# Arthur151/ROMP

Measured on NVIDIA H100. Metric: frames/sec 512x512 ROMP-HRNet32 (whole hot path), higher is better.
Workload: dtype bf16

## Files before the change

### romp_b200/_lib.py

```python
from __future__ import annotations

import ctypes as C
import os
import subprocess
import sys

HERE = os.path.dirname(os.path.abspath(__file__))
ROOT = os.path.dirname(HERE)
LIB_PATH = os.path.join(HERE, "lib", "libb200romp.so")
CSRC = os.path.join(HERE, "csrc")
SOURCES = ["net.cu", "conv_simt.cu", "conv_tc.cu", "conv_block_tc.cu", "conv_bottleneck_tc.cu", "conv_stem_tc.cu", "conv1d_tc.cu", "parse.cu", "smpl.cu", "smpl_blend_tc.cu", "project.cu", "pnp.cu", "bev.cu", "pack.cu", "preproc.cu", "temporal.cu", "track.cu", "romp_track.cu", "resnet_ops.cu"]

F32, BF16, U8 = 0, 1, 2
ENGINE_AUTO, ENGINE_SIMT, ENGINE_WGMMA, ENGINE_TF32 = 0, 1, 2, 3
ENGINE_TCGEN05 = ENGINE_WGMMA


class ConvDesc(C.Structure):
    _fields_ = [(n, C.c_int) for n in (
        "in_", "in_c_off", "out", "out_c_off", "res", "res_c_off", "res_broadcast", "cin", "cout",
        "ksize", "stride", "relu", "upsample", "input_norm", "pow_channel", "engine")]


class SumDesc(C.Structure):
    _fields_ = [("out", C.c_int), ("base", C.c_int), ("n_terms", C.c_int), ("term", C.c_int * 4), ("up", C.c_int * 4),
                ("relu", C.c_int), ("term_c_off", C.c_int * 4)]


class BevWeights(C.Structure):
    _fields_ = [(n, C.POINTER(C.c_float)) for n in (
        "center_ref", "cam_ref", "coordmap", "anchors", "embed", "w0", "b0", "w1", "b1", "w2", "b2")]


NVCC_FLAGS = ["-Xcompiler", "-fPIC", "-std=c++17", "-O3", "-lineinfo", "-gencode", "arch=compute_90a,code=sm_90a"]
OBJ_DIR = os.path.join(HERE, "lib", "obj")


def _nvcc():
    return os.environ.get("NVCC", "/usr/local/cuda/bin/nvcc")


def nvcc_command(out_path=LIB_PATH):
    return [_nvcc(), "-shared"] + NVCC_FLAGS + ["-o", out_path] + [os.path.join(CSRC, s) for s in SOURCES]


def _headers_mtime():
    hs = [os.path.join(CSRC, f) for f in os.listdir(CSRC) if f.endswith((".cuh", ".h"))]
    hs.append(os.path.join(ROOT, "include", "b200romp.h"))
    return max(os.path.getmtime(h) for h in hs)


def needs_build():
    if not os.path.exists(LIB_PATH):
        return True
    t = os.path.getmtime(LIB_PATH)
    deps = [os.path.join(CSRC, f) for f in os.listdir(CSRC)] + [os.path.join(ROOT, "include", "b200romp.h")]
    return any(os.path.getmtime(d) > t for d in deps)


def build(force=False, verbose=True):
    if not force and not needs_build():
        return LIB_PATH
    from concurrent.futures import ThreadPoolExecutor
    os.makedirs(OBJ_DIR, exist_ok=True)
# ... 143 lines not shown
```

### romp_b200/csrc/conv_tc.cuh

```cuda
#pragma once
#include <cuda.h>

#include <string>
#include <vector>

#include "common.cuh"

namespace b200romp {

struct S2Maps {
  CUtensorMap m[4];
};

struct TcConvPlan {
  int kind = 0;
  int cin = 0, cout = 0, nt = 0;
  int eb = 2;
  int grid_x = 0, grid_y = 0, stages = 0;
  int smem_bytes = 0;
  void* d_wpack = nullptr;
  CUtensorMap tmap_in;
  S2Maps tmap_s2;
  unsigned kmask = 0xFFFFFFFFu;
  const void* encoded_in = nullptr;
  int encoded_batch = 0;
  void* d_wpack2 = nullptr;
  void* d_wpack3 = nullptr;
  const float* d_bias1 = nullptr;
  const float* d_bias2 = nullptr;
  int fold = 0;
  std::string describe() const;
};

bool tc_conv_supported(const ConvParams& p, int ksize, int stride);
int tc_conv_prepare(const ConvParams& p, int ksize, int stride, const float* w_oihw, int sm_count, TcConvPlan* plan,
                    std::vector<void*>* allocs);
int tc_conv_launch(const TcConvPlan& plan, const ConvParams& p, cudaStream_t stream);
bool tc_conv1d_supported(const ConvParams& p);
int tc_conv1d_prepare(const ConvParams& p, const float* w_oi3, int sm_count, TcConvPlan* plan, std::vector<void*>* allocs);
int tc_conv1d_launch(TcConvPlan& plan, const ConvParams& p, cudaStream_t stream);
bool tc_stem_supported(const ConvParams& p, int ksize, int stride);
int tc_stem_prepare(const ConvParams& p, const float* w_oihw, int sm_count, TcConvPlan* plan, std::vector<void*>* allocs);
int tc_stem_launch(const TcConvPlan& plan, const ConvParams& p, cudaStream_t stream);
bool tc_block_supported(const ConvParams& p, bool fold);
int tc_block_prepare(const ConvParams& p, const float* w1_oihw, const float* b1, const float* w2_oihw, int sm_count,
                     TcConvPlan* plan, std::vector<void*>* allocs);
int tc_block_launch(const TcConvPlan& plan, const ConvParams& p, cudaStream_t stream);
struct BottleneckMids {
  __nv_bfloat16* t1 = nullptr;
  __nv_bfloat16* t2 = nullptr;
  int t1_C = 0, t2_C = 0;
};
bool tc_bottleneck_supported(const ConvParams& p);
int tc_bottleneck_prepare(const ConvParams& p, const float* w1_oihw, const float* b1, const float* w2_oihw, const float* b2,
                          const float* w3_oihw, int sm_count, TcConvPlan* plan, std::vector<void*>* allocs);
int tc_bottleneck_launch(const TcConvPlan& plan, const ConvParams& p, const BottleneckMids& mids, cudaStream_t stream);

}
```

### romp_b200/csrc/net.cu

```cuda
#include <stdarg.h>
#include <stdlib.h>
#include <string.h>

#include <algorithm>
#include <array>
#include <map>
#include <mutex>
#include <vector>

#include "common.cuh"
#include "conv_tc.cuh"

namespace b200romp {

static thread_local std::string g_last_error;

void set_error(const char* fmt, ...) {
  char buf[1024];
  va_list ap;
  va_start(ap, fmt);
  vsnprintf(buf, sizeof(buf), fmt, ap);
  va_end(ap);
  g_last_error = buf;
}

void* upload(const void* host, size_t bytes, std::vector<void*>* allocs) {
  void* d = nullptr;
  cudaError_t e = cudaMalloc(&d, bytes);
  if (e == cudaSuccess) {
    allocs->push_back(d);
    e = cudaMemcpy(d, host, bytes, cudaMemcpyHostToDevice);
  }
  if (e != cudaSuccess) {
    set_error("upload of %zu bytes failed: %s", bytes, cudaGetErrorString(e));
    return nullptr;
  }
  return d;
}

struct Tensor {
  int H, W, C, dtype, nchw, external;
  void* ptr = nullptr;
  bool constant = false;
  int first_def = -1, last_use = -1;
  size_t frame_bytes() const { return (size_t)H * W * C * dtype_size(dtype); }
};

enum class Kernel { Sum, MaxPool, Simt, Generic7x7, Deconv4x4, Wgmma, WgmmaStem, WgmmaConv1d, WgmmaBlock, WgmmaBottleneck };

struct Conv {
  b200romp_conv_desc d;
  std::vector<float> w, b;
  bool stored = false;
};

struct Op {
  Kernel kernel = Kernel::Simt;
  b200romp_sum_desc sum;
  b200romp_conv_desc d;
  std::vector<Conv> parts;
  float* d_w_simt = nullptr;
  float* d_bias = nullptr;
  int coutPad = 0;
  TcConvPlan tc;
  int lane = 0;
};

static std::vector<int> op_outputs(const Op& op) {
  std::vector<int> o{op.d.out};
  for (size_t k = 0; k + 1 < op.parts.size(); ++k)
    if (op.parts[k].stored) o.push_back(op.parts[k].d.out);
  return o;
}

static bool on_wgmma(Kernel k) {
  return k == Kernel::Wgmma || k == Kernel::WgmmaStem || k == Kernel::WgmmaConv1d || k == Kernel::WgmmaBlock || k == Kernel::WgmmaBottleneck;
}

}

using namespace b200romp;

struct b200romp_net {
  int device = 0;
  int sm_count = 132;
  bool finalized = false;
  int max_batch = 0;
  std::vector<Tensor> tensors;
  std::vector<Op> ops;
  std::vector<void*> device_allocs;
  char* workspace = nullptr;
  size_t workspace_bytes = 0;
  struct GraphKey {
    int batch;
    std::vector<void*> ext;
    bool operator<(const GraphKey& o) const { return batch != o.batch ? batch < o.batch : ext < o.ext; }
  };
  std::map<GraphKey, cudaGraphExec_t> graphs;
  bool use_graph = true;
  static constexpr int kLanes = 4;
  cudaStream_t lane_stream[kLanes] = {nullptr, nullptr, nullptr, nullptr};
  std::vector<cudaEvent_t> op_done;
  cudaEvent_t fork_ev = nullptr;
  bool use_lanes = false;
};

static int fill_params(const b200romp_net* net, const Op& op, int batch, bool allow_unbound, ConvParams* out) {
  const b200romp_conv_desc& d = op.d;
  const Tensor& ti = net->tensors[d.in];
  const Tensor& to = net->tensors[d.out];
  ConvParams p;
  memset(&p, 0, sizeof(p));
  p.in = ti.ptr; p.out = to.ptr;
  p.w = op.d_w_simt; p.bias = op.d_bias;
  p.B = batch;
  p.Hin = ti.H; p.Win = ti.W; p.in_C = ti.C; p.in_c_off = d.in_c_off; p.cin = d.cin;
  conv_out_hw(d.ksize, d.stride, ti.H, ti.W, &p.Hout, &p.Wout);
  p.out_C = to.C; p.out_c_off = d.out_c_off; p.cout = d.cout; p.coutPad = op.coutPad;
  p.up = d.upsample;
  if (d.res >= 0) {
    const Tensor& tr = net->tensors[d.res];
    p.res = tr.ptr; p.res_C = tr.C; p.res_c_off = op.d.res_c_off; p.res_broadcast = d.res_broadcast;
    p.res_dtype = tr.dtype;
  }
  p.relu = d.relu; p.pow_channel = d.pow_channel; p.out_nchw = to.nchw;
  p.in_dtype = ti.dtype; p.out_dtype = to.dtype; p.input_norm = d.input_norm;
  if (op.tc.fold) {
    p.Win /= 2; p.Wout /= 2;
    p.in_C *= 2; p.cin *= 2; p.out_C *= 2; p.cout *= 2; p.res_C *= 2;
  }
  if (!allow_unbound && (!p.in || !p.out)) {
    set_error("op uses an unbound tensor (in=%d out=%d)", d.in, d.out);
    return B200ROMP_ESTATE;
  }
  *out = p;
  return B200ROMP_OK;
}

static int validate_desc(const std::vector<Tensor>& T, const b200romp_conv_desc& d) {
  const int res_c_off = d.res_c_off;
  auto ok_id = [&](int id) { return id >= 0 && id < (int)T.size(); };
  B2R_REQUIRE(ok_id(d.in) && ok_id(d.out) && (d.res == -1 || ok_id(d.res)), "conv: bad tensor id");
  B2R_REQUIRE((d.ksize == 1 || d.ksize == 3 || d.ksize == 7 || (d.ksize == 13 && d.stride == 1 && d.upsample == 1) ||
               (d.ksize == 42 && d.stride == 2 && d.upsample == 1)) && (d.stride == 1 || d.stride == 2),
              "conv: ksize/stride unsupported");
  B2R_REQUIRE(d.upsample == 1 || d.upsample == 2 || d.upsample == 4 || d.upsample == 8, "conv: upsample must be 1,2,4,8");
  const Tensor& ti = T[d.in];
  const Tensor& to = T[d.out];
  B2R_REQUIRE(!ti.nchw, "conv: NCHW inputs unsupported");
  B2R_REQUIRE(d.cin > 0 && d.in_c_off >= 0 && d.in_c_off + d.cin <= ti.C, "conv: input channel slice out of range");
  B2R_REQUIRE(d.cout > 0 && d.out_c_off >= 0 && d.out_c_off + d.cout <= to.C, "conv: output channel slice out of range");
  int Ho, Wo;
  conv_out_hw(d.ksize, d.stride, ti.H, ti.W, &Ho, &Wo);
  B2R_REQUIRE(Ho * d.upsample == to.H && Wo * d.upsample == to.W, "conv: output tensor is %dx%d, op produces %dx%d",
              to.H, to.W, Ho * d.upsample, Wo * d.upsample);
  B2R_REQUIRE(ti.dtype != B200ROMP_U8 || d.input_norm || d.ksize == 7, "conv: u8 input requires input_norm (or the 7x7 stem)");
  B2R_REQUIRE(to.dtype != B200ROMP_U8, "conv: u8 output unsupported");
  B2R_REQUIRE(!to.nchw || to.dtype == B200ROMP_F32, "conv: NCHW output must be fp32");
  if (d.res >= 0) {
    const Tensor& tr = T[d.res];
    B2R_REQUIRE(tr.H == to.H && tr.W == to.W && !tr.nchw && tr.dtype != B200ROMP_U8, "conv: residual shape/dtype mismatch");
    B2R_REQUIRE(res_c_off >= 0 && res_c_off + d.cout <= tr.C, "conv: residual channel slice out of range");
  }
  return B200ROMP_OK;
}

extern "C" {

int b200romp_version(void) { return B200ROMP_VERSION; }
const char* b200romp_last_error(void) { return g_last_error.c_str(); }
// ... 112 lines not shown
  B2R_REQUIRE(to.H == (ti.H + 2 - 3) / 2 + 1 && to.W == (ti.W + 2 - 3) / 2 + 1, "add_maxpool: output must be %dx%d", (ti.H - 1) / 2 + 1, (ti.W - 1) / 2 + 1);
  Op op;
  op.kernel = Kernel::MaxPool;
  memset(&op.d, 0, sizeof(op.d));
  memset(&op.sum, 0, sizeof(op.sum));
  op.d.in = in; op.d.out = out; op.d.res = -1;
  net->ops.push_back(std::move(op));
  return (int)net->ops.size() - 1;
}

static int fill_sum_params(b200romp_net* net, const Op& op, int batch, SumParams* out) {
  SumParams p;
  memset(&p, 0, sizeof(p));
  const Tensor& to = net->tensors[op.sum.out];
  const Tensor& tb = net->tensors[op.sum.base];
  B2R_REQUIRE(to.ptr && tb.ptr, "sum op: unbound tensor");
  p.base = tb.ptr; p.base_dt = tb.dtype; p.out = to.ptr; p.out_dt = to.dtype;
  p.n_terms = op.sum.n_terms;
  for (int k = 0; k < p.n_terms; ++k) {
    const Tensor& tt = net->tensors[op.sum.term[k]];
    B2R_REQUIRE(tt.ptr, "sum op: unbound term tensor");
    p.term[k] = tt.ptr; p.term_dt[k] = tt.dtype; p.up[k] = op.sum.up[k];
    p.term_C[k] = tt.C; p.term_c_off[k] = op.sum.term_c_off[k];
  }
  p.B = batch; p.H = to.H; p.W = to.W; p.C = to.C; p.relu = op.sum.relu;
  *out = p;
  return B200ROMP_OK;
}

static int enqueue_op(b200romp_net* net, Op& op, int batch, cudaStream_t stream) {
  ConvParams p;
  if (op.kernel != Kernel::Sum && op.kernel != Kernel::MaxPool) {
    int rc = fill_params(net, op, batch, false, &p);
    if (rc) return rc;
  }
  switch (op.kernel) {
    case Kernel::Sum: {
      SumParams sp;
      int rc = fill_sum_params(net, op, batch, &sp);
      return rc ? rc : launch_fuse_sum(sp, stream);
    }
    case Kernel::MaxPool: {
      const Tensor& ti = net->tensors[op.d.in];
      const Tensor& to = net->tensors[op.d.out];
      B2R_REQUIRE(ti.ptr && to.ptr, "maxpool op: unbound tensor");
      return launch_maxpool3x3s2(ti.ptr, to.ptr, ti.dtype, batch, ti.H, ti.W, ti.C, stream);
    }
    case Kernel::Simt: return launch_conv_simt(p, op.d.ksize, op.d.stride, stream);
    case Kernel::Generic7x7: return launch_conv_generic(p, 7, op.d.stride, stream);
    case Kernel::Deconv4x4: return launch_deconv4x4s2(p, stream);
    case Kernel::Wgmma: return tc_conv_launch(op.tc, p, stream);
    case Kernel::WgmmaStem: return tc_stem_launch(op.tc, p, stream);
    case Kernel::WgmmaConv1d: return tc_conv1d_launch(op.tc, p, stream);
    case Kernel::WgmmaBlock: return tc_block_launch(op.tc, p, stream);
    case Kernel::WgmmaBottleneck: {
      BottleneckMids mids;
      auto mid = [&](int k, int* C) -> __nv_bfloat16* {
        if (!op.parts[k].stored) return nullptr;
        const Tensor& t = net->tensors[op.parts[k].d.out];
        *C = t.C;
        return static_cast<__nv_bfloat16*>(t.ptr);
      };
      mids.t1 = mid(0, &mids.t1_C);
      mids.t2 = mid(1, &mids.t2_C);
      return tc_bottleneck_launch(op.tc, p, mids, stream);
    }
  }
  return B200ROMP_EINVAL;
}

static bool fold_eligible(const b200romp_net* net, const Op& op) {
  static const bool off = [] { const char* e = getenv("B200ROMP_TC_NO_FOLD"); return e && e[0] == '1'; }();
  const b200romp_conv_desc& d = op.d;
  const Tensor& ti = net->tensors[d.in];
  const Tensor& to = net->tensors[d.out];
  if (off || d.ksize != 3 || d.stride != 1 || d.upsample != 1 || d.cin != 32 || d.cout != 32) return false;
  if (ti.C != 32 || to.C != 32 || d.in_c_off || d.out_c_off || ti.external || to.external) return false;
  if (ti.dtype != B200ROMP_BF16 || to.dtype != B200ROMP_BF16 || to.nchw || d.pow_channel >= 0 || d.input_norm) return false;
  if (ti.W % 16 != 0 || ti.H % 16 != 0) return false;
  if (d.res >= 0) {
    const Tensor& tr = net->tensors[d.res];
    if (tr.C != 32 || d.res_c_off || d.res_broadcast || tr.dtype != B200ROMP_BF16 || tr.external) return false;
  }
  return true;
}

static void fold_pixel_pairs(std::vector<float>* w, std::vector<float>* b) {
  std::vector<float> w2((size_t)64 * 64 * 9, 0.f), b2(64);
  for (int dx = 0; dx < 2; ++dx)
    for (int co = 0; co < 32; ++co)
      for (int h = 0; h < 2; ++h)
        for (int ci = 0; ci < 32; ++ci)
          for (int ky = 0; ky < 3; ++ky)
            for (int s = -1; s <= 1; ++s) {
              const int kx = 2 * s + h - dx + 1;
              if (kx < 0 || kx > 2) continue;
              w2[(((size_t)(dx * 32 + co) * 64 + h * 32 + ci) * 3 + ky) * 3 + (s + 1)] = (*w)[(((size_t)co * 32 + ci) * 3 + ky) * 3 + kx];
            }
  for (int i = 0; i < 64; ++i) b2[i] = (*b)[i % 32];
  *w = std::move(w2);
  *b = std::move(b2);
}

static unsigned fold_kmask() {
  unsigned m = 0;
  for (int t = 0; t < 9; ++t) {
    const int s = t % 3 - 1;
    if (s != -1) m |= 1u << (t * 2 + 0);
    if (s != +1) m |= 1u << (t * 2 + 1);
  }
  return m;
}

static bool is_bf16_relu_conv(const b200romp_net* net, const Op& op, int ksize, int cin, int cout) {
  const b200romp_conv_desc& d = op.d;
  const Tensor& ti = net->tensors[d.in];
  const Tensor& to = net->tensors[d.out];
  return d.ksize == ksize && d.stride == 1 && d.upsample == 1 && d.relu && !d.input_norm && d.pow_channel < 0 &&
         (d.engine == B200ROMP_ENGINE_AUTO || d.engine == B200ROMP_ENGINE_WGMMA) && ti.dtype == B200ROMP_BF16 &&
         to.dtype == B200ROMP_BF16 && !to.nchw && d.cin == cin && d.cout == cout;
}

static void count_accesses(const b200romp_net* net, std::vector<int>* reads, std::vector<int>* writes) {
  reads->assign(net->tensors.size(), 0);
  writes->assign(net->tensors.size(), 0);
  for (const Op& op : net->ops) {
    ++(*reads)[op.d.in];
    ++(*writes)[op.d.out];
    if (op.kernel == Kernel::Sum)
      for (int k = 0; k < op.sum.n_terms; ++k) ++(*reads)[op.sum.term[k]];
    else if (op.d.res >= 0) ++(*reads)[op.d.res];
  }
}

static bool fusable_intermediate(const b200romp_net* net, const Op& a, const Op& b, const std::vector<int>& writes) {
  const int t = a.d.out;
  const Tensor& tt = net->tensors[t];
  return b.d.in == t && b.d.in_c_off == 0 && a.d.out_c_off == 0 && tt.C == a.d.cout && !tt.external && !tt.constant &&
         writes[t] == 1 && b.d.res != t;
}

struct ChainPattern {
  Kernel kernel;
  std::vector<std::array<int, 3>> convs;
  bool fold;
  bool shared_mids;
  bool (*supported)(const ConvParams& p, bool fold);
};

static void fuse_chains(b200romp_net* net, const ChainPattern& pat) {
  std::vector<int> reads, writes;
  count_accesses(net, &reads, &writes);
  const size_t n = pat.convs.size();
  std::vector<Op> fused;
  fused.reserve(net->ops.size());
  for (size_t i = 0; i < net->ops.size(); ++i) {
    Op* c = &net->ops[i];
    bool ok = i + n <= net->ops.size();
    for (size_t k = 0; ok && k < n; ++k) {
      const std::array<int, 3>& s = pat.convs[k];
      ok = c[k].kernel == Kernel::Simt && is_bf16_relu_conv(net, c[k], s[0], s[1], s[2]) && c[k].lane == c[0].lane &&
           (!pat.fold || fold_eligible(net, c[k]));
      if (ok && k + 1 < n)
        ok = c[k].d.res < 0 && fusable_intermediate(net, c[k], c[k + 1], writes) && (pat.shared_mids || reads[c[k].d.out] == 1);
    }
    if (ok) {
      const b200romp_conv_desc& first = c[0].d;
      const b200romp_conv_desc& last = c[n - 1].d;
      ok = last.res == first.in && last.res_c_off == first.in_c_off && !last.res_broadcast &&
           !net->tensors[first.in].external && !net->tensors[last.out].external;
    }
    if (ok) {
      Op f;
      f.kernel = pat.kernel;
      f.d = c[0].d;
      f.d.cout = c[n - 1].d.cout;
      f.d.out = c[n - 1].d.out;
      f.d.out_c_off = c[n - 1].d.out_c_off;
      f.d.res = c[0].d.in;
      f.d.res_c_off = c[n - 1].d.res_c_off;
      f.tc.fold = pat.fold;
      f.lane = c[0].lane;
      ConvParams p;
      fill_params(net, f, 1, true, &p);
      if (pat.supported(p, pat.fold)) {
        for (size_t k = 0; k < n; ++k) {
          f.parts.push_back(std::move(c[k].parts[0]));
          f.parts.back().stored = k + 1 < n && reads[c[k].d.out] > 1;
        }
        fused.push_back(std::move(f));
        i += n - 1;
        continue;
      }
    }
    fused.push_back(std::move(net->ops[i]));
  }
  net->ops = std::move(fused);
}

static int choose_kernel(const b200romp_net* net, int i, Op& op) {
  const b200romp_conv_desc& d = op.d;
  const Tensor& ti = net->tensors[d.in];
  const Tensor& to = net->tensors[d.out];
  if (d.ksize == 7 || d.ksize == 42) {
    op.kernel = d.ksize == 7 ? Kernel::Generic7x7 : Kernel::Deconv4x4;
    return B200ROMP_OK;
  }
  op.kernel = Kernel::Simt;
  const bool forced = d.engine == B200ROMP_ENGINE_WGMMA;
  const bool stem = ti.dtype == B200ROMP_U8 && d.cin == 3 && d.ksize == 3 && d.stride == 2;
  if (!forced && !(d.engine == B200ROMP_ENGINE_TF32 && ti.dtype == B200ROMP_F32) &&
      !(d.engine == B200ROMP_ENGINE_AUTO && (ti.dtype == B200ROMP_BF16 || stem)))
    return B200ROMP_OK;
  ConvParams p;
  fill_params(net, op, net->max_batch, true, &p);
  if (stem) {
    if (!to.external && d.res < 0 && tc_stem_supported(p, d.ksize, d.stride)) op.kernel = Kernel::WgmmaStem;
  } else if (d.ksize == 13) {
    if (tc_conv1d_supported(p)) op.kernel = Kernel::WgmmaConv1d;
  } else if (!ti.external && tc_conv_supported(p, d.ksize, d.stride)) {
    op.kernel = Kernel::Wgmma;
    op.tc.fold = fold_eligible(net, op);
  }
  if (forced && op.kernel == Kernel::Simt) {
    set_error("op %d: tensor-core engine forced but shape unsupported", i);
    return B200ROMP_EINVAL;
  }
  return B200ROMP_OK;
}

static int prepare_op(b200romp_net* net, Op& op) {
  if (op.parts.empty()) return B200ROMP_OK;
  const b200romp_conv_desc& d = op.d;
  std::vector<std::vector<float>> w, b;
  for (Conv& c : op.parts) {
    w.push_back(std::move(c.w));
    b.push_back(std::move(c.b));
    if (op.tc.fold) fold_pixel_pairs(&w.back(), &b.back());
  }
  std::vector<float> bias = b.back();
  op.coutPad = ((int)bias.size() + 63) / 64 * 64;
  bias.resize(op.coutPad, 0.f);
  op.d_bias = static_cast<float*>(upload(bias.data(), bias.size() * sizeof(float), &net->device_allocs));
  if (!op.d_bias) return B200ROMP_ECUDA;
  ConvParams p;
  fill_params(net, op, net->max_batch, true, &p);
  switch (op.kernel) {
    case Kernel::Simt:
    case Kernel::Generic7x7:
    case Kernel::Deconv4x4: {
      const int taps = conv_taps(d.ksize);
      std::vector<float> packed((size_t)taps * d.cin * op.coutPad, 0.f);
      for (int co = 0; co < d.cout; ++co)
        for (int ci = 0; ci < d.cin; ++ci)
          for (int t = 0; t < taps; ++t)
            packed[((size_t)t * d.cin + ci) * op.coutPad + co] =
                d.ksize == 42 ? w[0][((size_t)ci * d.cout + co) * taps + t] : w[0][((size_t)co * d.cin + ci) * taps + t];
      op.d_w_simt = static_cast<float*>(upload(packed.data(), packed.size() * sizeof(float), &net->device_allocs));
      return op.d_w_simt ? B200ROMP_OK : B200ROMP_ECUDA;
    }
    case Kernel::Wgmma:
      if (op.tc.fold) op.tc.kmask = fold_kmask();
      return tc_conv_prepare(p, d.ksize, d.stride, w[0].data(), net->sm_count, &op.tc, &net->device_allocs);
    case Kernel::WgmmaStem: return tc_stem_prepare(p, w[0].data(), net->sm_count, &op.tc, &net->device_allocs);
    case Kernel::WgmmaConv1d: return tc_conv1d_prepare(p, w[0].data(), net->sm_count, &op.tc, &net->device_allocs);
    case Kernel::WgmmaBlock:
      return tc_block_prepare(p, w[0].data(), b[0].data(), w[1].data(), net->sm_count, &op.tc, &net->device_allocs);
    case Kernel::WgmmaBottleneck:
      return tc_bottleneck_prepare(p, w[0].data(), b[0].data(), w[1].data(), b[1].data(), w[2].data(), net->sm_count, &op.tc,
                                   &net->device_allocs);
    default: return B200ROMP_OK;
  }
}

int b200romp_net_finalize(b200romp_net* net, int max_batch) {
  B2R_REQUIRE(net && !net->finalized && max_batch > 0, "finalize: bad arguments");
  B2R_CUDA_OK(cudaSetDevice(net->device));
  fuse_chains(net, {Kernel::WgmmaBlock, {{3, 64, 64}, {3, 64, 64}}, false, false, tc_block_supported});
  fuse_chains(net, {Kernel::WgmmaBlock, {{3, 32, 32}, {3, 32, 32}}, true, false, tc_block_supported});
  fuse_chains(net, {Kernel::WgmmaBottleneck, {{1, 256, 64}, {3, 64, 64}, {1, 64, 256}}, false, true,
                    [](const ConvParams& p, bool) { return tc_bottleneck_supported(p); }});
  const int nT = (int)net->tensors.size(), nO = (int)net->ops.size();
  for (int i = 0; i < nO; ++i) {
    const b200romp_conv_desc& d = net->ops[i].d;
    for (int t : op_outputs(net->ops[i])) {
      Tensor& to = net->tensors[t];
      if (to.first_def < 0) to.first_def = i;
      to.last_use = std::max(to.last_use, i);
    }
    net->tensors[d.in].last_use = std::max(net->tensors[d.in].last_use, i);
    if (d.res >= 0) net->tensors[d.res].last_use = std::max(net->tensors[d.res].last_use, i);
    if (net->ops[i].kernel == Kernel::Sum)
      for (int k = 0; k < net->ops[i].sum.n_terms; ++k) {
        Tensor& tt = net->tensors[net->ops[i].sum.term[k]];
        B2R_REQUIRE(tt.external || tt.constant || (tt.first_def >= 0 && tt.first_def < i), "op %d sums tensor %d before it is written", i, net->ops[i].sum.term[k]);
        tt.last_use = std::max(tt.last_use, i);
      }
  }
  for (int i = 0; i < nO; ++i) {
    const b200romp_conv_desc& d = net->ops[i].d;
    const Tensor& ti = net->tensors[d.in];
    B2R_REQUIRE(ti.external || ti.constant || (ti.first_def >= 0 && ti.first_def < i), "op %d reads tensor %d before it is written", i, d.in);
    if (d.res >= 0) {
      const Tensor& tr = net->tensors[d.res];
      B2R_REQUIRE(tr.external || tr.constant || (tr.first_def >= 0 && tr.first_def < i), "op %d adds tensor %d before it is written", i, d.res);
    }
  }
  struct Buf { size_t bytes; size_t offset; };
  std::vector<Buf> bufs;
  std::multimap<size_t, int> free_bufs;
  std::vector<int> tensor_buf(nT, -1);
  std::vector<std::vector<int>> dies_at(nO);
  for (int t = 0; t < nT; ++t) {
    const Tensor& tt = net->tensors[t];
    if (!tt.external && !tt.constant && tt.first_def >= 0) dies_at[tt.last_use].push_back(t);
  }
  size_t total = 0;
  for (int i = 0; i < nO; ++i) {
    for (int t : op_outputs(net->ops[i])) {
      const Tensor& tt = net->tensors[t];
      if (tt.external || tt.constant || tt.first_def != i) continue;
      const size_t bytes = (tt.frame_bytes() * max_batch + 1023) / 1024 * 1024;
      auto it = free_bufs.find(bytes);
      if (it != free_bufs.end()) {
        tensor_buf[t] = it->second;
        free_bufs.erase(it);
      } else {
        bufs.push_back({bytes, total});
        total += bytes;
        tensor_buf[t] = (int)bufs.size() - 1;
      }
    }
    for (int dead : dies_at[i]) free_bufs.insert({bufs[tensor_buf[dead]].bytes, tensor_buf[dead]});
// ... 171 lines not shown
  const Tensor& t = net->tensors[tensor];
  B2R_REQUIRE(t.ptr != nullptr, "read_tensor: tensor %d has no storage", tensor);
  const size_t bytes = t.frame_bytes() * (t.constant ? 1 : batch);
  B2R_CUDA_OK(cudaMemcpyAsync(dst, t.ptr, bytes, cudaMemcpyDeviceToDevice, (cudaStream_t)stream));
  return B200ROMP_OK;
}

int b200romp_net_describe(b200romp_net* net, char* buf, int len) {
  if (!net || !buf || len <= 0) return B200ROMP_EINVAL;
  std::string s;
  char line[384];
  auto conv_line = [&](size_t i, const b200romp_conv_desc& d, Kernel kernel, const char* bracket) {
    const Tensor& ti = net->tensors[d.in];
    const Tensor& to = net->tensors[d.out];
    snprintf(line, sizeof(line), "op%03zu %s k%d s%d %4d->%-4d in t%d[%dx%dx%d]+%d out t%d[%dx%dx%d]+%d res t%d up%d relu%d%s\n", i,
             on_wgmma(kernel) ? "wgmma  " : "simt   ", d.ksize, d.stride, d.cin, d.cout, d.in, ti.H, ti.W, ti.C, d.in_c_off, d.out,
             to.H, to.W, to.C, d.out_c_off, d.res, d.upsample, d.relu, bracket);
    s += line;
  };
  for (size_t i = 0; i < net->ops.size(); ++i) {
    const Op& op = net->ops[i];
    const b200romp_conv_desc& d = op.d;
    const Tensor& ti = net->tensors[d.in];
    const Tensor& to = net->tensors[d.out];
    switch (op.kernel) {
      case Kernel::MaxPool:
        snprintf(line, sizeof(line), "op%03zu maxpool 3x3 s2 in t%d[%dx%dx%d] out t%d[%dx%dx%d]\n", i, d.in, ti.H, ti.W, ti.C, d.out, to.H, to.W, to.C);
        s += line;
        break;
      case Kernel::Sum: {
        int n = snprintf(line, sizeof(line), "op%03zu sum     out t%d[%dx%dx%d] = relu%d( t%d", i, op.sum.out, to.H, to.W, to.C, op.sum.relu, op.sum.base);
        for (int k = 0; k < op.sum.n_terms; ++k) n += snprintf(line + n, sizeof(line) - n, " + up%d(t%d)", op.sum.up[k], op.sum.term[k]);
        n += snprintf(line + n, sizeof(line) - n, " )");
        bool bound = net->finalized && to.ptr && ti.ptr;
        for (int k = 0; k < op.sum.n_terms; ++k) bound = bound && net->tensors[op.sum.term[k]].ptr;
        SumParams sp;
        if (bound && fill_sum_params(net, op, net->max_batch, &sp) == B200ROMP_OK)
          n += snprintf(line + n, sizeof(line) - n, " [fuse-sum %s]", fuse_sum_kernel_name(sp));
        snprintf(line + n, sizeof(line) - n, "\n");
        s += line;
        break;
      }
      case Kernel::WgmmaBlock: {
        const int mid = op.parts[0].d.out;
        const Tensor& tm = net->tensors[mid];
        snprintf(line, sizeof(line),
                 "op%03zu wgmma   block k3 s1 %d->%d->%d in t%d[%dx%dx%d]+%d mid t%d[%dx%dx%d] out t%d[%dx%dx%d]+%d res t%d+%d up1 relu1 "
                 "bias1 bias2 [tc-block grid %d smem %d%s]\n",
                 i, d.cin, d.cin, d.cout, d.in, ti.H, ti.W, ti.C, d.in_c_off, mid, tm.H, tm.W, tm.C, d.out, to.H, to.W, to.C,
                 d.out_c_off, d.res, d.res_c_off, op.tc.grid_x, op.tc.smem_bytes, op.tc.fold ? " conv1 pixel-pairs conv2 pixel-pairs" : "");
        s += line;
        break;
      }
      case Kernel::WgmmaBottleneck:
        for (size_t k = 0; k < op.parts.size(); ++k) {
          char bracket[96];
          snprintf(bracket, sizeof(bracket), " [tc-bottleneck conv%zu of k1-k3-k1 grid %d smem %d]", k + 1, op.tc.grid_x, op.tc.smem_bytes);
          conv_line(i, op.parts[k].d, op.kernel, bracket);
        }
        break;
      default:
        conv_line(i, d, op.kernel, on_wgmma(op.kernel) ? op.tc.describe().c_str() : "");
    }
  }
  snprintf(line, sizeof(line), "workspace %.1f MiB for max_batch %d\n", net->workspace_bytes / 1048576.0, net->max_batch);
  s += line;
  const int n = (int)std::min<size_t>(s.size(), (size_t)len - 1);
  memcpy(buf, s.data(), n);
  buf[n] = 0;
  return n;
}

int b200romp_net_set_lane(b200romp_net* net, int op, int lane) {
  B2R_REQUIRE(net && !net->finalized && op >= 0 && op < (int)net->ops.size(), "set_lane: bad op id or net already finalized");
  B2R_REQUIRE(lane >= 0 && lane < b200romp_net::kLanes, "set_lane: lane must be 0..%d", b200romp_net::kLanes - 1);
  net->ops[op].lane = lane;
  return B200ROMP_OK;
}

int b200romp_net_num_launches(b200romp_net* net) { return net ? (int)net->ops.size() : 0; }
long long b200romp_net_workspace_bytes(b200romp_net* net) { return net ? (long long)net->workspace_bytes : 0; }

int b200romp_conv2d(const b200romp_conv_desc* d, const float* weight_host, const float* bias_host, const void* in,
                    int in_dtype, int in_H, int in_W, int in_C, void* out, int out_dtype, int out_C, int out_nchw,
                    const void* res, int res_dtype, int batch, b200romp_stream stream) {
  B2R_REQUIRE(d && weight_host && in && out && batch > 0, "conv2d: bad arguments");
  int dev = 0;
  B2R_CUDA_OK(cudaGetDevice(&dev));
  b200romp_net* net = b200romp_net_create(dev);
  if (!net) return B200ROMP_ECUDA;
  int Ho, Wo;
  conv_out_hw(d->ksize, d->stride, in_H, in_W, &Ho, &Wo);
  Ho *= d->upsample; Wo *= d->upsample;
  b200romp_conv_desc dd = *d;
  dd.in = b200romp_net_add_tensor(net, in_H, in_W, in_C, in_dtype, 0, 1);
  dd.out = b200romp_net_add_tensor(net, Ho, Wo, out_C, out_dtype, out_nchw, 1);
  dd.res = -1;
  if (res) dd.res = b200romp_net_add_tensor(net, Ho, Wo, out_C, res_dtype, 0, 1);
  int rc = (dd.in < 0 || dd.out < 0) ? B200ROMP_EINVAL : B200ROMP_OK;
  if (!rc) {
    net->tensors[dd.in].ptr = const_cast<void*>(in);
    net->tensors[dd.out].ptr = out;
    if (res) net->tensors[dd.res].ptr = const_cast<void*>(res);
    net->tensors[dd.in].external = net->tensors[dd.out].external = 0;
    if (res) net->tensors[dd.res].external = 0;
    net->tensors[dd.in].constant = true;
// ... 24 lines not shown
```

Before: 3614.

## Fuse HRNet stem's two stride-2 3x3 convs into one warp-specialized WGMMA kernel

Adds a persistent kernel that loads raw u8 frames via TMA, normalizes and im2cols them in producer warps, runs conv1 (3->64, s2) with WGMMA into a parity-split shared-memory tile, then runs conv2 (64->64, s2) directly from shared memory. The aim is to avoid writing and re-reading the full-resolution 64-channel intermediate in global memory and to save a launch. The chain fuser is generalized to match stride, u8 input and non-residual patterns. The intermediate is still written out when another op reads it. This adds halo recomputation and a large shared-memory footprint that limits the kernel to one block per SM.

```diff
diff --git a/romp_b200/_lib.py b/romp_b200/_lib.py
--- a/romp_b200/_lib.py
+++ b/romp_b200/_lib.py
@@ -9,7 +9,7 @@
 ROOT = os.path.dirname(HERE)
 LIB_PATH = os.path.join(HERE, "lib", "libb200romp.so")
 CSRC = os.path.join(HERE, "csrc")
-SOURCES = ["net.cu", "conv_simt.cu", "conv_tc.cu", "conv_block_tc.cu", "conv_bottleneck_tc.cu", "conv_stem_tc.cu", "conv1d_tc.cu", "parse.cu", "smpl.cu", "smpl_blend_tc.cu", "project.cu", "pnp.cu", "bev.cu", "pack.cu", "preproc.cu", "temporal.cu", "track.cu", "romp_track.cu", "resnet_ops.cu"]
+SOURCES = ["net.cu", "conv_simt.cu", "conv_tc.cu", "conv_block_tc.cu", "conv_bottleneck_tc.cu", "conv_stem_tc.cu", "conv_stem_fused_tc.cu", "conv1d_tc.cu", "parse.cu", "smpl.cu", "smpl_blend_tc.cu", "project.cu", "pnp.cu", "bev.cu", "pack.cu", "preproc.cu", "temporal.cu", "track.cu", "romp_track.cu", "resnet_ops.cu"]
 
 F32, BF16, U8 = 0, 1, 2
 ENGINE_AUTO, ENGINE_SIMT, ENGINE_WGMMA, ENGINE_TF32 = 0, 1, 2, 3
diff --git a/romp_b200/csrc/conv_stem_fused_tc.cu b/romp_b200/csrc/conv_stem_fused_tc.cu
--- /dev/null
+++ b/romp_b200/csrc/conv_stem_fused_tc.cu
@@ -0,0 +1,337 @@
+#include "conv_tc.cuh"
+#include "tc_device.cuh"
+
+namespace b200romp {
+
+namespace {
+
+constexpr int kFsThreads = 384;
+constexpr int kFsRowB = 128;
+constexpr int kFsK1RowB = 64;
+constexpr int kFsMidRows = 576;
+constexpr int kFsW2Bytes = 9 * 64 * kFsRowB;
+constexpr int kFsMidBytes = kFsMidRows * kFsRowB;
+constexpr int kFsA1Bytes = kFsMidRows * kFsK1RowB;
+constexpr int kFsW1Bytes = 64 * kFsK1RowB;
+constexpr int kFsRawRowB = 112;
+constexpr int kFsRawRows = 67;
+constexpr int kFsRawBytes = kFsRawRowB * kFsRawRows;
+constexpr int kFsRawStage = (kFsRawBytes + 127) / 128 * 128;
+constexpr int kFsRing = 2;
+constexpr int kFsSmemBytes = kFsW2Bytes + kFsMidBytes + kFsA1Bytes + kFsW1Bytes + kFsRing * kFsRawStage + 1024  +
+                             1024 ;
+static_assert(kFsSmemBytes <= 227 * 1024, "fused stem does not fit shared memory");
+
+__host__ __device__ constexpr int fs_bh(int i) { return i < 2 ? 17 : 16; }
+__host__ __device__ constexpr int fs_bw(int i) { return (i & 1) ? 8 : 9; }
+__host__ __device__ constexpr int fs_sub_row(int i) { return i == 0 ? 0 : fs_sub_row(i - 1) + (fs_bh(i - 1) * fs_bw(i - 1) + 7) / 8 * 8; }
+static_assert(fs_sub_row(4) == 568, "parity layout rows");
+
+__device__ __forceinline__ bool fs_row(int m, int* yl, int* xl) {
+  const int i = m < fs_sub_row(1) ? 0 : m < fs_sub_row(2) ? 1 : m < fs_sub_row(3) ? 2 : 3;
+  const int r = m - (i == 0 ? fs_sub_row(0) : i == 1 ? fs_sub_row(1) : i == 2 ? fs_sub_row(2) : fs_sub_row(3));
+  const int bw = fs_bw(i), a = r / bw, b = r % bw;
+  const bool ok = m < fs_sub_row(4) && a < fs_bh(i);
+  *yl = ok ? 2 * a + (i < 2 ? 0 : 1) : 0;
+  *xl = ok ? 2 * b + ((i & 1) ? 1 : 0) : 0;
+  return ok;
+}
+
+__device__ __forceinline__ void consumers_bar_sync() { asm volatile("bar.sync 1, 256;" ::: "memory"); }
+
+template <typename T>
+__device__ __forceinline__ T opaque(T v) {
+  uint64_t u = (uint64_t)v;
+  asm volatile("mov.b64 %0, %0;" : "+l"(u));
+  return (T)u;
+}
+__device__ __forceinline__ void stmatrix_x4(uint32_t addr, uint32_t r0, uint32_t r1, uint32_t r2, uint32_t r3) {
+  asm volatile("stmatrix.sync.aligned.m8n8.x4.shared.b16 [%0], {%1, %2, %3, %4};" ::"r"(addr), "r"(r0), "r"(r1), "r"(r2), "r"(r3)
+               : "memory");
+}
+__device__ __forceinline__ uint32_t pack_bf16x2(float a, float b) {
+  const __nv_bfloat162 v = __floats2bfloat162_rn(a, b);
+  return *reinterpret_cast<const uint32_t*>(&v);
+}
+
+}
+
+template <bool STORE_MID>
+__global__ void __launch_bounds__(kFsThreads, 1)
+conv_stem_fused_tc_kernel(const __grid_constant__ CUtensorMap raw_map, const ConvParams p, const uint8_t* __restrict__ w1pack,
+                          const uint8_t* __restrict__ w2pack, const float* __restrict__ bias1, __nv_bfloat16* __restrict__ mid,
+                          int tiles_x, int tiles_y, int num_tiles) {
+  extern __shared__ uint8_t smem_raw[];
+  uint8_t* smem = reinterpret_cast<uint8_t*>((reinterpret_cast<uintptr_t>(smem_raw) + 1023) & ~(uintptr_t)1023);
+  uint8_t* sW2 = smem;
+  uint8_t* sMid = sW2 + kFsW2Bytes;
+  uint8_t* sA1 = sMid + kFsMidBytes;
+  uint8_t* sW1 = sA1 + kFsA1Bytes;
+  uint8_t* sRaw = sW1 + kFsW1Bytes;
+  uint64_t* raw_full = reinterpret_cast<uint64_t*>(sRaw + kFsRing * kFsRawStage);
+  uint64_t* raw_empty = raw_full + kFsRing;
+  uint64_t* w_full = raw_empty + kFsRing;
+  uint64_t* a1_full = w_full + 1;
+  uint64_t* a1_empty = a1_full + 1;
+
+  const int warp = threadIdx.x >> 5, l = threadIdx.x & 31;
+  if (threadIdx.x == 0) {
+    for (int i = 0; i < kFsRing; ++i) {
+      mbar_init(&raw_full[i], 1);
+      mbar_init(&raw_empty[i], 3);
+    }
+    mbar_init(w_full, 1);
+    mbar_init(a1_full, 3);
+    mbar_init(a1_empty, 8);
+    fence_barrier_init();
+  }
+  __syncthreads();
+  pdl_trigger();
+  const int per_frame = tiles_x * tiles_y;
+
+  if (warp == 0) {
+    if (elect_one()) {
+      mbar_arrive_expect_tx(w_full, kFsW1Bytes + kFsW2Bytes);
+      bulk_copy_g2s(sW1, w1pack, kFsW1Bytes, w_full);
+      for (int t = 0; t < 9; ++t) bulk_copy_g2s(sW2 + t * 64 * kFsRowB, w2pack + (size_t)t * 64 * kFsRowB, 64 * kFsRowB, w_full);
+      pdl_wait();
+      const uint64_t pol = l2_policy_stream();
+      int slot = 0;
+      uint32_t phase = 0;
+      for (int tile = blockIdx.x; tile < num_tiles; tile += gridDim.x) {
+        const int n = tile / per_frame, rem = tile % per_frame;
+        const int y0 = (rem / tiles_x) * 16, x0 = (rem % tiles_x) * 8;
+        mbar_wait(&raw_empty[slot], phase ^ 1);
+        mbar_arrive_expect_tx(&raw_full[slot], kFsRawBytes);
+        tma_load_3d(sRaw + slot * kFsRawStage, &raw_map, &raw_full[slot], 12 * x0 - 16, 4 * y0 - 3, n, pol);
+        if (++slot == kFsRing) { slot = 0; phase ^= 1; }
+      }
+    }
+  } else if (warp < 4) {
+    const int pt = threadIdx.x - 32;
+    int slot = 0;
+    uint32_t phase = 0, it = 0;
+    for (int tile = blockIdx.x; tile < num_tiles; tile += gridDim.x, ++it) {
+      const int rem = tile % per_frame;
+      const int y0 = (rem / tiles_x) * 16, x0 = (rem % tiles_x) * 8;
+      mbar_wait(&raw_full[slot], phase);
+      mbar_wait(a1_empty, (it & 1) ^ 1);
+      const uint8_t* raw = sRaw + slot * kFsRawStage;
+#pragma unroll 1
+      for (int m = pt; m < kFsMidRows; m += 96) {
+        int yl, xl;
+        const bool row_valid = fs_row(m, &yl, &xl);
+        const int off = 2 * yl * kFsRawRowB + 7 + 6 * xl;
+        const uint32_t* src = reinterpret_cast<const uint32_t*>(raw + (off & ~3));
+        const int sh = 8 * (off & 3);
+        float v[32];
+#pragma unroll
+        for (int r = 0; r < 3; ++r) {
+          const int iy = 4 * y0 - 3 + 2 * yl + r;
+          const bool row_ok = row_valid && iy >= 0 && iy < p.Hin;
+          const uint32_t* q = src + r * (kFsRawRowB / 4);
+          const uint32_t a0 = q[0], a1 = q[1], a2 = q[2];
+          const uint32_t b[3] = {__funnelshift_r(a0, a1, sh), __funnelshift_r(a1, a2, sh), a2 >> sh};
+#pragma unroll
+          for (int s = 0; s < 3; ++s) {
+            const int ix = 4 * x0 - 3 + 2 * xl + s;
+            const bool ok = row_ok && ix >= 0 && ix < p.Win;
+#pragma unroll
+            for (int c = 0; c < 3; ++c) {
+              const int k = s * 3 + c;
+              const float x = __uint_as_float(__byte_perm(b[k >> 2], 0x4B000000u, 0x7540u | (k & 3)));
+              v[r * 9 + k] = ok ? (x - 8388608.f) - 127.5f : 0.f;
+            }
+          }
+        }
+#pragma unroll
+        for (int k = 27; k < 32; ++k) v[k] = 0.f;
+        uint32_t pk[16];
+#pragma unroll
+        for (int k = 0; k < 16; ++k) pk[k] = pack_bf16x2(v[2 * k], v[2 * k + 1]);
+        uint8_t* a = sA1 + m * kFsK1RowB;
+#pragma unroll
+        for (int q4 = 0; q4 < 4; ++q4)
+          *reinterpret_cast<uint4*>(a + ((q4 ^ ((m >> 1) & 3)) * 16)) = make_uint4(pk[4 * q4], pk[4 * q4 + 1], pk[4 * q4 + 2], pk[4 * q4 + 3]);
+      }
+      fence_proxy_async();
+      __syncwarp();
+      if (l == 0) {
+        mbar_arrive(a1_full);
+        mbar_arrive(&raw_empty[slot]);
+      }
+      if (++slot == kFsRing) { slot = 0; phase ^= 1; }
+    }
+  } else {
+    const int g = (warp >> 2) - 1, w = warp & 3;
+    pdl_wait();
+    mbar_wait(w_full, 0);
+    const int cl = 2 * (l & 3);
+    const int Hmid = 2 * p.Hout, Wmid = 2 * p.Wout;
+    uint32_t it = 0;
+    for (int tile = blockIdx.x; tile < num_tiles; tile += gridDim.x, ++it) {
+      const uint32_t w1_base = opaque(smem_u32(sW1)), w2_base = opaque(smem_u32(sW2)), a1_base = opaque(smem_u32(sA1)),
+                     mid_base = opaque(smem_u32(sMid));
+      const float* b1p = opaque(bias1);
+      const float* b2p = opaque(p.bias);
+      const int n = tile / per_frame, rem = tile % per_frame;
+      const int y0 = (rem / tiles_x) * 16, x0 = (rem % tiles_x) * 8;
+
+      auto issue64 = [&](float (&acc)[32], int blk) {
+        wgmma_fence();
+#pragma unroll
+        for (int k = 0; k < 2; ++k)
+          wgmma_n64(acc, make_smem_desc(a1_base + blk * 64 * kFsK1RowB + k * 32, 8 * kFsK1RowB, kSw64),
+                    make_smem_desc(w1_base + k * 32, 8 * kFsK1RowB, kSw64), k, false);
+        wgmma_commit();
+      };
+      float b1v[16], b1h[8];
+#pragma unroll
+      for (int j = 0; j < 8; ++j) { b1v[2 * j] = __ldg(b1p + 8 * j + cl); b1v[2 * j + 1] = __ldg(b1p + 8 * j + cl + 1); }
+#pragma unroll
+      for (int j = 0; j < 4; ++j) { b1h[2 * j] = __ldg(b1p + 32 * g + 8 * j + cl); b1h[2 * j + 1] = __ldg(b1p + 32 * g + 8 * j + cl + 1); }
+      auto epi = [&](const auto& acc, const auto& bias, int blk, int j0) {
+        constexpr int NJ = sizeof(acc) / (4 * sizeof(float));
+        bool zero[2];
+        size_t gpix[2];
+        bool store[2];
+#pragma unroll
+        for (int e = 0; e < 2; ++e) {
+          int yl, xl;
+          const bool row_valid = fs_row(blk * 64 + 16 * w + (l >> 2) + 8 * e, &yl, &xl);
+          const int my = 2 * y0 - 1 + yl, mx = 2 * x0 - 1 + xl;
+          zero[e] = !row_valid || (unsigned)my >= (unsigned)Hmid || (unsigned)mx >= (unsigned)Wmid;
+          store[e] = row_valid && yl >= 1 && xl >= 1;
+          gpix[e] = ((size_t)n * Hmid + my) * Wmid + mx;
+        }
+        const int q = l >> 3, rr = l & 7;
+        const uint32_t row_addr = mid_base + (uint32_t)((blk * 64 + 16 * w + rr + 8 * (q & 1)) * kFsRowB);
+#pragma unroll
+        for (int j = 0; j < NJ; j += 2) {
+          uint32_t r[4];
+#pragma unroll
+          for (int qq = 0; qq < 4; ++qq) {
+            const int e = qq & 1, jl = j + (qq >> 1), jg = j0 + jl;
+            const float a = fmaxf(acc[4 * jl + 2 * e] + bias[2 * jl], 0.f), b = fmaxf(acc[4 * jl + 2 * e + 1] + bias[2 * jl + 1], 0.f);
+            r[qq] = zero[e] ? 0u : pack_bf16x2(a, b);
+            if constexpr (STORE_MID) {
+              if (store[e]) *reinterpret_cast<uint32_t*>(mid + gpix[e] * 64 + 8 * jg + cl) = r[qq];
+            }
+          }
+          stmatrix_x4(row_addr + (((j0 + j + (q >> 1)) ^ rr) << 4), r[0], r[1], r[2], r[3]);
+        }
+      };
+      float acc0[32], acc1[32], acc_b[16];
+      mbar_wait(a1_full, it & 1);
+      issue64(acc0, 4 * g);
+      issue64(acc1, 4 * g + 1);
+      wgmma_wait<1>();
+      consumers_bar_sync();
+      epi(acc0, b1v, 4 * g, 0);
+      issue64(acc0, 4 * g + 2);
+      wgmma_wait<1>();
+      epi(acc1, b1v, 4 * g + 1, 0);
+      issue64(acc1, 4 * g + 3);
+      wgmma_wait<1>();
+      epi(acc0, b1v, 4 * g + 2, 0);
+      wgmma_fence();
+#pragma unroll
+      for (int k = 0; k < 2; ++k)
+        wgmma_n32(acc_b, make_smem_desc(a1_base + 8 * 64 * kFsK1RowB + k * 32, 8 * kFsK1RowB, kSw64),
+                  make_smem_desc(w1_base + 32 * g * kFsK1RowB + k * 32, 8 * kFsK1RowB, kSw64), k, false);
+      wgmma_commit();
+      wgmma_wait<1>();
+      epi(acc1, b1v, 4 * g + 3, 0);
+      wgmma_wait<0>();
+      if (l == 0) mbar_arrive(a1_empty);
+      epi(acc_b, b1h, 8, 4 * g);
+      fence_proxy_async();
+      consumers_bar_sync();
+
+      float acc2[32];
+#pragma unroll
+      for (int j = 0; j < 32; ++j) acc2[j] = 0.f;
+      wgmma_fence();
+#pragma unroll
+      for (int tap = 0; tap < 9; ++tap) {
+        const int r = tap / 3, s = tap % 3;
+        const int sub = (r != 1 ? 0 : 2) + (s != 1 ? 0 : 1);
+        const int bw = fs_bw(sub);
+        const uint32_t a_tap = mid_base + (uint32_t)((fs_sub_row(sub) + (r == 2 ? bw : 0) + (s == 2 ? 1 : 0) + 8 * g * bw) * kFsRowB);
+        const uint32_t b_tap = w2_base + (uint32_t)(tap * 64 * kFsRowB);
+#pragma unroll
+        for (int k = 0; k < 4; ++k)
+          wgmma_n64(acc2, make_smem_desc(a_tap + k * 32, bw * kFsRowB, kSw128), make_smem_desc(b_tap + k * 32, 8 * kFsRowB, kSw128),
+                    (tap | k) != 0, false);
+      }
+      wgmma_commit();
+      wgmma_wait<0>();
+
+      __nv_bfloat16* out = reinterpret_cast<__nv_bfloat16*>(p.out);
+#pragma unroll
+      for (int e = 0; e < 2; ++e) {
+        const size_t pix = ((size_t)n * p.Hout + y0 + 8 * g + 2 * w + e) * p.Wout + x0 + (l >> 2);
+        __nv_bfloat162* o = reinterpret_cast<__nv_bfloat162*>(out + pix * p.out_C + p.out_c_off + cl);
+#pragma unroll
+        for (int j = 0; j < 8; ++j) {
+          const int c = 8 * j + cl;
+          o[4 * j] = __floats2bfloat162_rn(fmaxf(acc2[4 * j + 2 * e] + __ldg(b2p + c), 0.f),
+                                           fmaxf(acc2[4 * j + 2 * e + 1] + __ldg(b2p + c + 1), 0.f));
+        }
+      }
+    }
+  }
+}
+
+bool tc_stem_fused_supported(const ConvParams& p) {
+  return p.cin == 3 && p.in_C == 3 && p.in_c_off == 0 && p.cout == 64 && p.in_dtype == B200ROMP_U8 && p.input_norm &&
+         p.out_dtype == B200ROMP_BF16 && !p.out_nchw && p.up == 1 && p.res == nullptr && p.relu && p.pow_channel < 0 &&
+         p.out_C % 8 == 0 && p.out_c_off % 8 == 0 && p.Hout % 16 == 0 && p.Wout % 8 == 0 && p.Hout * 4 == p.Hin &&
+         p.Wout * 4 == p.Win && (p.Win * 3) % 16 == 0;
+}
+
+int tc_stem_fused_prepare(const ConvParams& p, const float* w1_oihw, const float* b1, const float* w2_oihw, int sm_count,
+                          TcConvPlan* plan, std::vector<void*>* allocs) {
+  plan->kind = 34;
+  plan->eb = 2;
+  plan->cin = 3;
+  plan->cout = plan->nt = 64;
+  plan->grid_x = sm_count;
+  plan->grid_y = 1;
+  plan->stages = kFsRing;
+  plan->smem_bytes = kFsSmemBytes;
+  std::vector<float> wk((size_t)64 * 32, 0.f);
+  for (int co = 0; co < 64; ++co)
+    for (int c = 0; c < 3; ++c)
+      for (int r = 0; r < 3; ++r)
+        for (int s = 0; s < 3; ++s)
+          wk[(size_t)co * 32 + r * 9 + s * 3 + c] = w1_oihw[(((size_t)co * 3 + c) * 3 + r) * 3 + s] * (2.0f / 255.0f);
+  int rc = tc_pack_weights(wk.data(), 32, 64, 1, 64, &plan->d_wpack, allocs, kFsK1RowB, 2);
+  if (!rc) rc = tc_pack_weights(w2_oihw, 64, 64, 9, 64, &plan->d_wpack2, allocs, kFsRowB, 2);
+  if (rc) return rc;
+  plan->d_bias1 = static_cast<const float*>(upload(b1, 64 * sizeof(float), allocs));
+  if (!plan->d_bias1) return B200ROMP_ECUDA;
+  B2R_CUDA_OK(cudaFuncSetAttribute(conv_stem_fused_tc_kernel<false>, cudaFuncAttributeMaxDynamicSharedMemorySize, kFsSmemBytes));
+  B2R_CUDA_OK(cudaFuncSetAttribute(conv_stem_fused_tc_kernel<true>, cudaFuncAttributeMaxDynamicSharedMemorySize, kFsSmemBytes));
+  return B200ROMP_OK;
+}
+
+int tc_stem_fused_launch(const TcConvPlan& plan, const ConvParams& p, __nv_bfloat16* mid, cudaStream_t stream) {
+  B2R_REQUIRE((reinterpret_cast<uintptr_t>(p.in) & 15) == 0 && (p.Win * 3) % 16 == 0,
+              "conv_stem_fused_tc: frames must be 16 B aligned with a row pitch that is a multiple of 16 B");
+  CUtensorMap raw;
+  const cuuint64_t gdim[3] = {(cuuint64_t)p.Win * 3, (cuuint64_t)p.Hin, (cuuint64_t)p.B};
+  const cuuint64_t gstr[2] = {(cuuint64_t)p.Win * 3, (cuuint64_t)p.Win * 3 * p.Hin};
+  const cuuint32_t box[3] = {(cuuint32_t)kFsRawRowB, (cuuint32_t)kFsRawRows, 1};
+  if (tc_encode_tiled(&raw, CU_TENSOR_MAP_DATA_TYPE_UINT8, 3, p.in, gdim, gstr, box, CU_TENSOR_MAP_SWIZZLE_NONE, "conv_stem_fused_tc (frames)"))
+    return B200ROMP_EINVAL;
+  const int tiles_x = p.Wout / 8, tiles_y = p.Hout / 16;
+  const int num_tiles = tiles_x * tiles_y * p.B;
+  const dim3 grid(std::min(plan.grid_x, num_tiles));
+  auto kern = mid != nullptr ? conv_stem_fused_tc_kernel<true> : conv_stem_fused_tc_kernel<false>;
+  B2R_CUDA_OK(tc_launch(kern, grid, kFsThreads, plan.smem_bytes, stream, raw, p, reinterpret_cast<const uint8_t*>(plan.d_wpack),
+                        reinterpret_cast<const uint8_t*>(plan.d_wpack2), plan.d_bias1, mid, tiles_x, tiles_y, num_tiles));
+  return B200ROMP_OK;
+}
+
+}
diff --git a/romp_b200/csrc/conv_tc.cuh b/romp_b200/csrc/conv_tc.cuh
--- a/romp_b200/csrc/conv_tc.cuh
+++ b/romp_b200/csrc/conv_tc.cuh
@@ -42,6 +42,10 @@
 bool tc_stem_supported(const ConvParams& p, int ksize, int stride);
 int tc_stem_prepare(const ConvParams& p, const float* w_oihw, int sm_count, TcConvPlan* plan, std::vector<void*>* allocs);
 int tc_stem_launch(const TcConvPlan& plan, const ConvParams& p, cudaStream_t stream);
+bool tc_stem_fused_supported(const ConvParams& p);
+int tc_stem_fused_prepare(const ConvParams& p, const float* w1_oihw, const float* b1, const float* w2_oihw, int sm_count,
+                          TcConvPlan* plan, std::vector<void*>* allocs);
+int tc_stem_fused_launch(const TcConvPlan& plan, const ConvParams& p, __nv_bfloat16* mid, cudaStream_t stream);
 bool tc_block_supported(const ConvParams& p, bool fold);
 int tc_block_prepare(const ConvParams& p, const float* w1_oihw, const float* b1, const float* w2_oihw, int sm_count,
                      TcConvPlan* plan, std::vector<void*>* allocs);
diff --git a/romp_b200/csrc/net.cu b/romp_b200/csrc/net.cu
--- a/romp_b200/csrc/net.cu
+++ b/romp_b200/csrc/net.cu
@@ -46,7 +46,7 @@
   size_t frame_bytes() const { return (size_t)H * W * C * dtype_size(dtype); }
 };
 
-enum class Kernel { Sum, MaxPool, Simt, Generic7x7, Deconv4x4, Wgmma, WgmmaStem, WgmmaConv1d, WgmmaBlock, WgmmaBottleneck };
+enum class Kernel { Sum, MaxPool, Simt, Generic7x7, Deconv4x4, Wgmma, WgmmaStem, WgmmaConv1d, WgmmaStemFused, WgmmaBlock, WgmmaBottleneck };
 
 struct Conv {
   b200romp_conv_desc d;
@@ -74,7 +74,8 @@
 }
 
 static bool on_wgmma(Kernel k) {
-  return k == Kernel::Wgmma || k == Kernel::WgmmaStem || k == Kernel::WgmmaConv1d || k == Kernel::WgmmaBlock || k == Kernel::WgmmaBottleneck;
+  return k == Kernel::Wgmma || k == Kernel::WgmmaStem || k == Kernel::WgmmaConv1d || k == Kernel::WgmmaStemFused || k == Kernel::WgmmaBlock ||
+         k == Kernel::WgmmaBottleneck;
 }
 
 }
@@ -115,7 +116,7 @@
   p.w = op.d_w_simt; p.bias = op.d_bias;
   p.B = batch;
   p.Hin = ti.H; p.Win = ti.W; p.in_C = ti.C; p.in_c_off = d.in_c_off; p.cin = d.cin;
-  conv_out_hw(d.ksize, d.stride, ti.H, ti.W, &p.Hout, &p.Wout);
+  p.Hout = to.H / d.upsample; p.Wout = to.W / d.upsample;
   p.out_C = to.C; p.out_c_off = d.out_c_off; p.cout = d.cout; p.coutPad = op.coutPad;
   p.up = d.upsample;
   if (d.res >= 0) {
@@ -334,6 +335,10 @@
     case Kernel::Wgmma: return tc_conv_launch(op.tc, p, stream);
     case Kernel::WgmmaStem: return tc_stem_launch(op.tc, p, stream);
     case Kernel::WgmmaConv1d: return tc_conv1d_launch(op.tc, p, stream);
+    case Kernel::WgmmaStemFused: {
+      const Tensor& tm = net->tensors[op.parts[0].d.out];
+      return tc_stem_fused_launch(op.tc, p, op.parts[0].stored ? static_cast<__nv_bfloat16*>(tm.ptr) : nullptr, stream);
+    }
     case Kernel::WgmmaBlock: return tc_block_launch(op.tc, p, stream);
     case Kernel::WgmmaBottleneck: {
       BottleneckMids mids;
@@ -394,13 +399,13 @@
   return m;
 }
 
-static bool is_bf16_relu_conv(const b200romp_net* net, const Op& op, int ksize, int cin, int cout) {
+static bool is_relu_conv(const b200romp_net* net, const Op& op, const std::array<int, 4>& s, bool u8_in) {
   const b200romp_conv_desc& d = op.d;
   const Tensor& ti = net->tensors[d.in];
   const Tensor& to = net->tensors[d.out];
-  return d.ksize == ksize && d.stride == 1 && d.upsample == 1 && d.relu && !d.input_norm && d.pow_channel < 0 &&
-         (d.engine == B200ROMP_ENGINE_AUTO || d.engine == B200ROMP_ENGINE_WGMMA) && ti.dtype == B200ROMP_BF16 &&
-         to.dtype == B200ROMP_BF16 && !to.nchw && d.cin == cin && d.cout == cout;
+  return d.ksize == s[0] && d.stride == s[1] && d.upsample == 1 && d.relu && d.input_norm == (u8_in ? 1 : 0) && d.pow_channel < 0 &&
+         (d.engine == B200ROMP_ENGINE_AUTO || d.engine == B200ROMP_ENGINE_WGMMA) &&
+         ti.dtype == (u8_in ? B200ROMP_U8 : B200ROMP_BF16) && to.dtype == B200ROMP_BF16 && !to.nchw && d.cin == s[2] && d.cout == s[3];
 }
 
 static void count_accesses(const b200romp_net* net, std::vector<int>* reads, std::vector<int>* writes) {
@@ -424,9 +429,11 @@
 
 struct ChainPattern {
   Kernel kernel;
-  std::vector<std::array<int, 3>> convs;
+  std::vector<std::array<int, 4>> convs;
   bool fold;
   bool shared_mids;
+  bool residual;
+  bool u8_input;
   bool (*supported)(const ConvParams& p, bool fold);
 };
 
@@ -440,8 +447,7 @@
     Op* c = &net->ops[i];
     bool ok = i + n <= net->ops.size();
     for (size_t k = 0; ok && k < n; ++k) {
-      const std::array<int, 3>& s = pat.convs[k];
-      ok = c[k].kernel == Kernel::Simt && is_bf16_relu_conv(net, c[k], s[0], s[1], s[2]) && c[k].lane == c[0].lane &&
+      ok = c[k].kernel == Kernel::Simt && is_relu_conv(net, c[k], pat.convs[k], pat.u8_input && k == 0) && c[k].lane == c[0].lane &&
            (!pat.fold || fold_eligible(net, c[k]));
       if (ok && k + 1 < n)
         ok = c[k].d.res < 0 && fusable_intermediate(net, c[k], c[k + 1], writes) && (pat.shared_mids || reads[c[k].d.out] == 1);
@@ -449,8 +455,8 @@
     if (ok) {
       const b200romp_conv_desc& first = c[0].d;
       const b200romp_conv_desc& last = c[n - 1].d;
-      ok = last.res == first.in && last.res_c_off == first.in_c_off && !last.res_broadcast &&
-           !net->tensors[first.in].external && !net->tensors[last.out].external;
+      ok = (pat.residual ? last.res == first.in && last.res_c_off == first.in_c_off && !last.res_broadcast : last.res < 0) &&
+           (pat.u8_input || !net->tensors[first.in].external) && !net->tensors[last.out].external;
     }
     if (ok) {
       Op f;
@@ -459,8 +465,8 @@
       f.d.cout = c[n - 1].d.cout;
       f.d.out = c[n - 1].d.out;
       f.d.out_c_off = c[n - 1].d.out_c_off;
-      f.d.res = c[0].d.in;
-      f.d.res_c_off = c[n - 1].d.res_c_off;
+      f.d.res = pat.residual ? c[0].d.in : -1;
+      f.d.res_c_off = pat.residual ? c[n - 1].d.res_c_off : 0;
       f.tc.fold = pat.fold;
       f.lane = c[0].lane;
       ConvParams p;
@@ -546,6 +552,8 @@
       return tc_conv_prepare(p, d.ksize, d.stride, w[0].data(), net->sm_count, &op.tc, &net->device_allocs);
     case Kernel::WgmmaStem: return tc_stem_prepare(p, w[0].data(), net->sm_count, &op.tc, &net->device_allocs);
     case Kernel::WgmmaConv1d: return tc_conv1d_prepare(p, w[0].data(), net->sm_count, &op.tc, &net->device_allocs);
+    case Kernel::WgmmaStemFused:
+      return tc_stem_fused_prepare(p, w[0].data(), b[0].data(), w[1].data(), net->sm_count, &op.tc, &net->device_allocs);
     case Kernel::WgmmaBlock:
       return tc_block_prepare(p, w[0].data(), b[0].data(), w[1].data(), net->sm_count, &op.tc, &net->device_allocs);
     case Kernel::WgmmaBottleneck:
@@ -558,9 +566,11 @@
 int b200romp_net_finalize(b200romp_net* net, int max_batch) {
   B2R_REQUIRE(net && !net->finalized && max_batch > 0, "finalize: bad arguments");
   B2R_CUDA_OK(cudaSetDevice(net->device));
-  fuse_chains(net, {Kernel::WgmmaBlock, {{3, 64, 64}, {3, 64, 64}}, false, false, tc_block_supported});
-  fuse_chains(net, {Kernel::WgmmaBlock, {{3, 32, 32}, {3, 32, 32}}, true, false, tc_block_supported});
-  fuse_chains(net, {Kernel::WgmmaBottleneck, {{1, 256, 64}, {3, 64, 64}, {1, 64, 256}}, false, true,
+  fuse_chains(net, {Kernel::WgmmaStemFused, {{3, 2, 3, 64}, {3, 2, 64, 64}}, false, true, false, true,
+                    [](const ConvParams& p, bool) { return tc_stem_fused_supported(p); }});
+  fuse_chains(net, {Kernel::WgmmaBlock, {{3, 1, 64, 64}, {3, 1, 64, 64}}, false, false, true, false, tc_block_supported});
+  fuse_chains(net, {Kernel::WgmmaBlock, {{3, 1, 32, 32}, {3, 1, 32, 32}}, true, false, true, false, tc_block_supported});
+  fuse_chains(net, {Kernel::WgmmaBottleneck, {{1, 1, 256, 64}, {3, 1, 64, 64}, {1, 1, 64, 256}}, false, true, true, false,
                     [](const ConvParams& p, bool) { return tc_bottleneck_supported(p); }});
   const int nT = (int)net->tensors.size(), nO = (int)net->ops.size();
   for (int i = 0; i < nO; ++i) {
@@ -838,6 +848,14 @@
         s += line;
         break;
       }
+      case Kernel::WgmmaStemFused:
+        for (size_t k = 0; k < op.parts.size(); ++k) {
+          char bracket[128];
+          snprintf(bracket, sizeof(bracket), " [tc k3 v%d nt64 grid %dx1 smem %d stages %d] [tc-stem conv%zu of k3s2-k3s2]", k == 0 ? 3 : 2,
+                   op.tc.grid_x, op.tc.smem_bytes, op.tc.stages, k + 1);
+          conv_line(i, op.parts[k].d, op.kernel, bracket);
+        }
+        break;
       case Kernel::WgmmaBottleneck:
         for (size_t k = 0; k < op.parts.size(); ++k) {
           char bracket[96];
```

After: 3664, median of 6. 1.01x the previous value.
